# refresh-bio/colord

Hardware: AMD Instinct MI355X
Metric: input Gbases/s + archive size vs ref, ONT 50 Gb at 1/2/4/8 MI355X (higher is better)
Workload: dtype u64

## Files before the change

### colord_amd/csrc/dna.hip

```cpp
#include "common.hpp"
#include <functional>
#include "objects.hpp"
#include "rc_dev.hpp"
#include "rc_check.hpp"
#include "es_format.hpp"
#include <algorithm>
#include <deque>
#include <thread>
#include <chrono>

namespace {
enum { F_READ_TYPE = 0, F_REV_COMP, F_SEEN, F_LEN_BITS, F_LEN_DATA, F_SYMBOLS, F_SYMBOLS_N, F_READ_ID, F_READ_ID_SHORT,
       F_ANCHOR_LEN, F_SKIP_LOCAL, F_SKIP_DISTANT, F_TUPLE_TYPE, N_FAM };
constexpr uint32_t MAX_ALT = 64;

struct FamTab {
	uint32_t n_sym[N_FAM], max_total[N_FAM], adder[N_FAM];
	uint32_t ctx_base[N_FAM + 1];
	uint64_t state_base[N_FAM + 1];
	uint32_t n_ctx[N_FAM];
	int32_t level, T, S;
	uint32_t sym_B;
	uint32_t max_alt;
	uint32_t long_run;
	uint32_t walk_chunk, walk_warm;
};

struct RefStore { const uint64_t* packed; const uint64_t* word_off; const uint32_t* lens; uint32_t n; };
__device__ inline uint32_t ref_at(const RefStore& R, uint32_t id, bool rev, int64_t pos)
{
	if (id >= R.n) return 255;
	const uint32_t len = R.lens[id];
	if (pos < 0 || pos >= (int64_t)len) return 255;
	const uint32_t p = rev ? (len - 1 - (uint32_t)pos) : (uint32_t)pos;
	const uint32_t b = (uint32_t)(R.packed[R.word_off[id] + (p >> 5)] >> (62 - 2 * (p & 31))) & 3u;
	return rev ? 3u - b : b;
}
struct RefCur {
	uint32_t id = 0xffffffffu, len = 0, widx = 0xffffffffu; bool rev = false, ok = false; uint64_t wo = 0, word = 0;
	__device__ inline void set(const RefStore& R, uint32_t nid, bool nrev)
	{
		rev = nrev;
		if (nid == id) return;
		id = nid; widx = 0xffffffffu; ok = nid < R.n;
		if (ok) { len = R.lens[nid]; wo = R.word_off[nid]; }
	}
	__device__ inline uint32_t at(const RefStore& R, int64_t pos)
	{
		if (!ok || pos < 0 || pos >= (int64_t)len) return 255;
		const uint32_t p = rev ? (len - 1 - (uint32_t)pos) : (uint32_t)pos;
		if ((p >> 5) != widx) { widx = p >> 5; word = R.packed[wo + widx]; }
		const uint32_t b = (uint32_t)(word >> (62 - 2 * (p & 31))) & 3u;
		return rev ? 3u - b : b;
	}
};
__device__ inline uint32_t ilog2_(uint64_t x) { return x ? 64u - (uint32_t)__clzll((long long)x) : 0u; }
__device__ inline uint32_t no_bytes_(uint64_t x) { uint32_t r = 1; x >>= 8; for (; x; ++r) x >>= 8; return r; }

template<typename K> struct KeyFmt {
	static __host__ __device__ inline K make(uint32_t gctx, uint32_t payload) { return ((K)gctx << 8) | (K)payload; }
	static __host__ __device__ inline uint32_t ctx(K k) { return (uint32_t)(k >> 8); }
	static __host__ __device__ inline uint32_t payload(K k) { return (uint32_t)k & 0xffu; }
};
__device__ inline uint32_t key_payload(int fam, uint32_t sym, int e1, int e2)
{
	if (fam == F_TUPLE_TYPE)
	{
		const uint32_t x = e1 == 15 ? 0u : e2 == 15 ? (e1 == T_ANCHOR ? 1u : 2u) : e1 == T_ANCHOR ? 3u : e1 == T_DEL ? 4u : 5u;
		return (x << 3) | sym;
	}
	if (fam == F_SYMBOLS) return ((e1 == 15 ? 0u : (uint32_t)e1 + 1u) << 2) | sym;
	return sym;
}
__device__ inline void key_decode(uint32_t fam, uint32_t p, uint32_t& sym, uint32_t& e1, uint32_t& e2)
{
	if (fam == F_TUPLE_TYPE)
	{
		const uint32_t x = p >> 3; sym = p & 7u;
		e1 = x == 0 ? 15u : (x == 1 || x == 3) ? (uint32_t)T_ANCHOR : x == 2 ? (uint32_t)T_SKIP : x == 4 ? (uint32_t)T_DEL : (uint32_t)T_ALT_ID;
		e2 = x == 3 ? (uint32_t)T_MATCH : x == 4 ? (uint32_t)T_SKIP : x == 5 ? (uint32_t)T_MAIN_REF : 15u;
	}
	else if (fam == F_SYMBOLS) { const uint32_t x = p >> 2; sym = p & 3u; e1 = x ? x - 1u : 15u; e2 = 15u; }
	else { sym = p; e1 = e2 = 15u; }
}
__device__ inline uint32_t key_sym_mask(uint32_t fam) { return fam == F_TUPLE_TYPE ? 7u : fam == F_SYMBOLS ? 3u : 0xffu; }

// ... 372 lines not shown
	if (r >= r1) return;
	uint32_t t = es[es_off[r]] >> 4;
	flag[r - r0] = t == T_START_PLAIN ? 0 : t == T_START_PLAIN_N ? 1 : 2;
}

__global__ __launch_bounds__(256) void k_fill_sidx(const uint64_t* __restrict__ sym_off, uint64_t s0, uint32_t r0, uint32_t r1, TripLayoutDev lay, uint32_t* __restrict__ sidx)
{
	const uint32_t r = r0 + blockIdx.x * 4 + (threadIdx.x >> 6);
	if (r >= r1) return;
	const uint32_t lane = threadIdx.x & 63;
	const uint64_t a = sym_off[r] - s0, b = sym_off[r + 1] - s0;
	if (a == b) return;
	const uint32_t part = part_of_read(lay, r), pl = lay.rank ? lay.rank[part] : part;
	const uint64_t gb = lay.group_base[pl >> 6], p0 = lay.part_sym_start[part];
	for (uint64_t i = a + lane; i < b; i += 64) sidx[i] = (uint32_t)trip_slot(gb, pl & 63, i - p0);
}
template<typename K>
__global__ __launch_bounds__(256) void k_dna_plain(const FamTab* __restrict__ ftp, const uint8_t* __restrict__ es, const uint64_t* __restrict__ es_off,
                                                  const uint32_t* __restrict__ es_ntup, const uint8_t* __restrict__ read_flag, const uint32_t* __restrict__ hdr_counts,
                                                  const uint64_t* __restrict__ sym_off, uint32_t r0, uint32_t r1, K* __restrict__ key)
{
	const uint32_t r = r0 + blockIdx.x * 4 + (threadIdx.x >> 6);
	if (r >= r1) return;
	const uint32_t fl = read_flag[r - r0];
	if (fl == 2) return;
	const FamTab& ft = *ftp;
	const uint32_t lane = threadIdx.x & 63;
	const uint8_t* b = es + es_off[r] + 1;
	const uint32_t len = es_ntup[r] - 1;
	const uint64_t off = sym_off[r - r0] + hdr_counts[r - r0];
	const uint32_t S2 = 2 * ft.S; const uint32_t mask = (1u << S2) - 1;
	const uint32_t fam = fl == 0 ? F_SYMBOLS : F_SYMBOLS_N;
	const uint32_t cbase = ft.ctx_base[fam];
	for (uint32_t i = lane; i < len; i += 64)
	{
		uint32_t ctx = mask;
		if (fl == 0)
		{
			const uint32_t n = i < (uint32_t)ft.S ? i : (uint32_t)ft.S;
			for (uint32_t t = n; t >= 1; --t) ctx = ((ctx << 2) + (b[i - t] & 3u)) & mask;
			ctx <<= 2;
		}
		else
		{
			const uint32_t n = i < 4 ? i : 4;
			for (uint32_t t = n; t >= 1; --t) ctx = ((ctx << 4) + (b[i - t] & 0xfu)) & mask;
		}
		key[off + i] = KeyFmt<K>::make(cbase + ctx, b[i] & 0xfu);
	}
}


constexpr uint32_t LONG_RUN = 1u << 19;
struct LongRun { uint32_t s, e, fam, gctx; uint64_t step0, group0, epoch0; uint32_t epoch_cap, pad; };
template<int NS> struct EpochRec { uint32_t start, tot; uint32_t st[NS]; uint32_t cnt0[NS]; };
__device__ inline uint32_t find_run(const LongRun* runs, uint32_t n_runs, uint64_t step)
{
	uint32_t lo = 0, hi = n_runs;
	while (hi - lo > 1) { const uint32_t mid = (lo + hi) >> 1; if (runs[mid].step0 <= step) lo = mid; else hi = mid; }
	return lo;
}
template<typename K>
__global__ void k_long_find(const uint32_t* __restrict__ seg_start, uint32_t n_seg, const K* __restrict__ skey, const FamTab* __restrict__ ftp, LongRun* __restrict__ runs , uint32_t cap, uint32_t* __restrict__ n_runs )
{
	const uint32_t sg = blockIdx.x * blockDim.x + threadIdx.x;
	if (sg >= n_seg) return;
	const uint32_t s = seg_start[sg], e = seg_start[sg + 1];
	const FamTab& ft = *ftp;
	if (e - s < ft.long_run) return;
	const uint32_t gctx = KeyFmt<K>::ctx(skey[s]);
	uint32_t fam = 0;
	for (uint32_t f = 1; f < N_FAM; ++f) if (gctx >= ft.ctx_base[f]) fam = f;
	if (ft.n_sym[fam] > 32) return;
	const uint32_t which = ft.n_sym[fam] > 8 ? 1u : 0u;
	const uint32_t i = atomicAdd(n_runs + which, 1u);
	if (i < cap) { LongRun r; r.s = s; r.e = e; r.fam = fam; r.gctx = gctx; r.step0 = r.group0 = r.epoch0 = 0; r.epoch_cap = 0; r.pad = 0; runs[which * cap + i] = r; }
}
template<int NS, typename K>
__global__ __launch_bounds__(256) void k_long_hist(const LongRun* __restrict__ runs, uint32_t n_runs, uint64_t n_groups, const K* __restrict__ skey,
                                                  uint32_t* __restrict__ step_pfx, uint32_t* __restrict__ group_tot)
{
	const uint64_t g = ((uint64_t)blockIdx.x * blockDim.x + threadIdx.x) >> 6; const uint32_t lane = threadIdx.x & 63;
	if (g >= n_groups) return;
	uint32_t lo = 0, hi = n_runs;
	while (hi - lo > 1) { const uint32_t mid = (lo + hi) >> 1; if (runs[mid].group0 <= g) lo = mid; else hi = mid; }
	const LongRun R = runs[lo];
	const uint64_t gl = g - R.group0;
	const uint32_t smask = key_sym_mask(R.fam);
	uint32_t c[NS];
#pragma unroll
	for (int a = 0; a < NS; ++a) c[a] = 0;
	for (uint32_t k = 0; k < 64; ++k)
	{
		const uint64_t j = (uint64_t)R.s + (gl * 64 + k) * 64 + lane;
		const bool valid = j < R.e;
		const uint32_t sym = valid ? (uint32_t)skey[j] & smask : 0xffu;
#pragma unroll
		for (uint32_t a = 0; a < NS; ++a) { const uint32_t n = (uint32_t)__popcll(__ballot(sym == a)); if (lane == k) c[a] = n; }
	}
	const uint64_t n_steps = ((uint64_t)(R.e - R.s) + 63) / 64;
	const uint64_t step = R.step0 + gl * 64 + lane;
#pragma unroll
	for (uint32_t a = 0; a < NS; ++a)
	{
		const uint32_t incl = wave_incl_scan(c[a]);
		if (gl * 64 + lane < n_steps) step_pfx[step * NS + a] = incl - c[a];
		if (lane == 63) group_tot[g * NS + a] = incl;
	}
}
template<int NS>
__global__ __launch_bounds__(64) void k_long_groups(const LongRun* __restrict__ runs, uint32_t n_runs, uint32_t* __restrict__ group_tot )
{
	const uint32_t r = blockIdx.x, lane = threadIdx.x;
	if (r >= n_runs) return;
	const LongRun R = runs[r];
	const uint64_t n_steps = ((uint64_t)(R.e - R.s) + 63) / 64, n_groups = (n_steps + 63) / 64;
	uint32_t carry[NS];
#pragma unroll
	for (int a = 0; a < NS; ++a) carry[a] = 0;
	for (uint64_t g0 = 0; g0 < n_groups; g0 += 64)
	{
		const uint64_t g = g0 + lane; const bool valid = g < n_groups;
#pragma unroll
		for (uint32_t a = 0; a < NS; ++a)
		{
			const uint32_t v = valid ? group_tot[(R.group0 + g) * NS + a] : 0u;
			const uint32_t incl = wave_incl_scan(v);
			if (valid) group_tot[(R.group0 + g) * NS + a] = carry[a] + incl - v;
			carry[a] += __shfl(incl, 63);
		}
	}
}
template<int NS, typename K>
__device__ inline uint32_t long_prefix(const LongRun& R, const K* skey, const uint32_t* step_pfx, const uint32_t* group_pfx, uint32_t x, uint32_t lane)
{
	const uint32_t smask = key_sym_mask(R.fam);
	const uint64_t step = x >> 6; const uint32_t off = x & 63;
	const uint32_t a = lane & (NS - 1);
	uint32_t v = group_pfx[(R.group0 + (step >> 6)) * NS + a] + (step * 64 < (uint64_t)(R.e - R.s) || off ? step_pfx[(R.step0 + step) * NS + a] : 0u);
	if (x == R.e - R.s && off == 0)
	{
		const uint64_t last = step - 1;
		const uint64_t j = (uint64_t)R.s + last * 64 + lane; const uint32_t sym = j < R.e ? (uint32_t)skey[j] & smask : 0xffu;
		uint32_t mine = 0;
#pragma unroll
		for (uint32_t b = 0; b < NS; ++b) { const uint32_t n = (uint32_t)__popcll(__ballot(sym == b)); if (a == b) mine = n; }
		return group_pfx[(R.group0 + (last >> 6)) * NS + a] + step_pfx[(R.step0 + last) * NS + a] + mine;
	}
	if (off)
	{
		const uint64_t j = (uint64_t)R.s + step * 64 + lane; const uint32_t sym = j < R.e ? (uint32_t)skey[j] & smask : 0xffu;
		const uint64_t below = (1ULL << off) - 1;
		uint32_t mine = 0;
#pragma unroll
		for (uint32_t b = 0; b < NS; ++b) { const uint32_t n = (uint32_t)__popcll(__ballot(sym == b) & below); if (a == b) mine = n; }
		v += mine;
	}
	return v;
}
template<int NS, typename K>
__global__ __launch_bounds__(64) void k_long_epochs(const FamTab* __restrict__ ftp, const LongRun* __restrict__ runs, uint32_t n_runs, const K* __restrict__ skey,
                                                   const uint32_t* __restrict__ step_pfx, const uint32_t* __restrict__ group_pfx, uint32_t* __restrict__ state,
                                                   EpochRec<NS>* __restrict__ epochs, uint32_t* __restrict__ n_epochs, uint32_t* __restrict__ group_epoch, uint32_t* __restrict__ err)
{
	const uint32_t r = blockIdx.x, lane = threadIdx.x;
	if (r >= n_runs) return;
	const LongRun R = runs[r];
	const FamTab& ft = *ftp;
	const uint32_t n_sym = ft.n_sym[R.fam], max_total = ft.max_total[R.fam], adder = ft.adder[R.fam];
	uint32_t* sp = state + ft.state_base[R.fam] + (uint64_t)(R.gctx - ft.ctx_base[R.fam]) * (n_sym + 1);
	const uint32_t L = R.e - R.s;
	uint32_t st = lane < n_sym ? sp[lane] : 0u, tot = sp[n_sym];
	uint32_t cnt0 = 0, p = 0, ne = 0;
	EpochRec<NS>* E = epochs + R.epoch0;
	for (;;)
	{
		if (ne >= R.epoch_cap) { if (lane == 0) atomicOr(err, 8u); break; }
		if (lane < NS) { E[ne].st[lane] = st; E[ne].cnt0[lane] = cnt0; }
		if (lane == 0) { E[ne].start = p; E[ne].tot = tot; }
		++ne;
		const uint32_t rr = (max_total - tot + adder - 1) / adder;
		if ((uint64_t)p + rr > L) break;
		p += rr;
		const uint32_t c1 = long_prefix<NS, K>(R, skey, step_pfx, group_pfx, p, lane);
		st += adder * (c1 - cnt0); cnt0 = c1;
		tot += adder * rr;
		while (tot >= max_total)
		{
			st = (st + 1) / 2;
			uint32_t sm = lane < NS ? st : 0u;
			for (int o = NS / 2; o; o >>= 1) sm += __shfl_xor(sm, o);
			tot = __shfl(sm, 0);
		}
		if (p == L) { if (lane < NS && ne < R.epoch_cap) { E[ne].st[lane] = st; E[ne].cnt0[lane] = cnt0; } if (lane == 0 && ne < R.epoch_cap) { E[ne].start = p; E[ne].tot = tot; } ++ne; break; }
	}
	const uint32_t cl = long_prefix<NS, K>(R, skey, step_pfx, group_pfx, L, lane);
	if (p < L) { st += adder * (cl - cnt0); tot += adder * (L - p); }
	if (lane < n_sym) sp[lane] = st;
	if (lane == 0) { sp[n_sym] = tot; n_epochs[r] = ne; }
	__builtin_amdgcn_s_waitcnt(0);
	__builtin_amdgcn_fence(__ATOMIC_SEQ_CST, "workgroup");
	const uint64_t n_groups = (((uint64_t)L + 63) / 64 + 63) / 64;
	for (uint64_t g0 = 0; g0 < n_groups; g0 += 64)
	{
		const uint64_t g = g0 + lane;
		if (g >= n_groups) continue;
		const uint32_t pos = (uint32_t)(g * 4096);
		uint32_t lo = 0, hi = ne;
		while (hi - lo > 1) { const uint32_t mid = (lo + hi) >> 1; if (E[mid].start <= pos) lo = mid; else hi = mid; }
		group_epoch[R.group0 + g] = lo;
	}
}
template<int NS, typename K>
__global__ __launch_bounds__(256) void k_long_apply(const LongRun* __restrict__ runs, uint32_t n_runs, uint64_t n_steps, const K* __restrict__ skey, const uint32_t* __restrict__ sval,
                                                   const uint32_t* __restrict__ step_pfx, const uint32_t* __restrict__ group_pfx, const EpochRec<NS>* __restrict__ epochs,
                                                   const uint32_t* __restrict__ n_epochs, const uint32_t* __restrict__ group_epoch, const FamTab* __restrict__ ftp, triple_t* __restrict__ trip)
{
	const uint64_t step = ((uint64_t)blockIdx.x * blockDim.x + threadIdx.x) >> 6; const uint32_t lane = threadIdx.x & 63;
	if (step >= n_steps) return;
	const uint32_t ri = find_run(runs, n_runs, step);
	const LongRun R = runs[ri];
	const uint32_t adder = ftp->adder[R.fam];
	const uint64_t sl = step - R.step0;
	const uint32_t x0 = (uint32_t)(sl * 64), x = x0 + lane;
	const uint64_t j = (uint64_t)R.s + x; const bool valid = j < R.e;
	uint32_t sym = 0xffu, e1 = 15u, e2 = 15u;
	if (valid) key_decode(R.fam, KeyFmt<K>::payload(skey[j]), sym, e1, e2);
	uint64_t m[NS];
#pragma unroll
	for (uint32_t a = 0; a < NS; ++a) m[a] = __ballot(sym == a);
	const EpochRec<NS>* E = epochs + R.epoch0; const uint32_t ne = n_epochs[ri];
	uint32_t e = group_epoch[R.group0 + (sl >> 6)];
	while (e + 1 < ne && E[e + 1].start <= x0) ++e;
	uint32_t me = e;
	while (me + 1 < ne && E[me + 1].start <= x) ++me;
	if (!valid) return;
	const EpochRec<NS>& ep = E[me];
	const uint64_t lt = (1ULL << lane) - 1;
	uint32_t cum = 0, freq = 0, excl = 0;
#pragma unroll
	for (uint32_t a = 0; a < NS; ++a)
	{
		const uint32_t pre = group_pfx[(R.group0 + (sl >> 6)) * NS + a] + step_pfx[step * NS + a] + (uint32_t)__popcll(m[a] & lt);
		const uint32_t v = ep.st[a] + adder * (pre - ep.cnt0[a]);
		const bool ex = NS <= 8 && (a == e1 || a == e2);
		if (ex) excl += v;
		if (a < sym && !ex) cum += v;
		if (a == sym) freq = v;
	}
	trip[sval[j]] = pack_triple(cum, freq, ep.tot + adder * (x - ep.start) - excl);
}

template<typename K>
__global__ __launch_bounds__(256) void k_dna_evolve(const FamTab* __restrict__ ftp, const K* __restrict__ skey, const uint32_t* __restrict__ sval,
                                                   const uint32_t* __restrict__ seg_start, uint32_t n_seg, uint32_t* __restrict__ state, triple_t* __restrict__ trip)
{
	__shared__ uint32_t s_cnt[4][256];
	__shared__ uint32_t s_pre[4][256];
	const uint32_t w = threadIdx.x >> 6, lane = threadIdx.x & 63;
	const uint32_t sg = blockIdx.x * 4 + w;
	if (sg >= n_seg) return;
	const uint32_t s = seg_start[sg], e = seg_start[sg + 1];
	const FamTab& ft = *ftp;
	const uint32_t gctx = KeyFmt<K>::ctx(skey[s]);
	uint32_t fam = 0;
	for (uint32_t f = 1; f < N_FAM; ++f) if (gctx >= ft.ctx_base[f]) fam = f;
	const uint32_t n_sym = ft.n_sym[fam], max_total = ft.max_total[fam], adder = ft.adder[fam];
	uint32_t* sp = state + ft.state_base[fam] + (uint64_t)(gctx - ft.ctx_base[fam]) * (n_sym + 1);
	const uint64_t lt = (1ULL << lane) - 1;
	if (n_sym <= 8)
	{
		if (e - s >= ft.long_run) return;
		uint32_t st[8]; uint32_t tot = sp[n_sym];
#pragma unroll
		for (uint32_t a = 0; a < 8; ++a) st[a] = a < n_sym ? sp[a] : 0u;
		for (uint32_t j0 = s; j0 < e; j0 += 64)
		{
			const uint32_t j = j0 + lane; const bool valid = j < e;
			uint32_t sym = 0xffu, e1 = 15u, e2 = 15u;
			if (valid) key_decode(fam, KeyFmt<K>::payload(skey[j]), sym, e1, e2);
			const uint32_t dst = valid ? sval[j] : 0u;
			uint64_t m[8];
#pragma unroll
			for (uint32_t a = 0; a < 8; ++a) m[a] = __ballot(valid && sym == a);
			const uint32_t cnt = (e - j0) < 64 ? (e - j0) : 64;
			uint32_t start = 0;
			while (start < cnt)
			{
				const uint32_t r = (max_total - tot + adder - 1) / adder;
				const uint32_t now = (cnt - start) < r ? (cnt - start) : r;
				const uint64_t win = (now == 64 ? ~0ULL : ((1ULL << now) - 1)) << start;
				if (lane >= start && lane < start + now)
				{
					const uint64_t before = lt & win;
					uint32_t cum = 0, freq = 0, excl = 0;
#pragma unroll
					for (uint32_t a = 0; a < 8; ++a)
					{
						const uint32_t v = st[a] + adder * (uint32_t)__popcll(m[a] & before);
						const bool ex = a == e1 || a == e2;
						if (ex) excl += v;
						if (a < sym && !ex) cum += v;
						if (a == sym) freq = v;
					}
					trip[dst] = pack_triple(cum, freq, tot + adder * (lane - start) - excl);
				}
#pragma unroll
				for (uint32_t a = 0; a < 8; ++a) st[a] += adder * (uint32_t)__popcll(m[a] & win);
				tot += adder * now;
				while (tot >= max_total)
				{
					tot = 0;
#pragma unroll
					for (uint32_t a = 0; a < 8; ++a) { st[a] = (st[a] + 1) / 2; tot += st[a]; }
				}
				start += now;
			}
		}
		if (lane == 0)
		{
			for (uint32_t a = 0; a < n_sym; ++a) sp[a] = st[a];
			sp[n_sym] = tot;
		}
		return;
	}
	if (n_sym <= 32 && e - s >= ft.long_run) return;
	uint32_t* cnt = s_cnt[w]; uint32_t* pre = s_pre[w];
#pragma unroll
	for (uint32_t t = 0; t < 4; ++t) { uint32_t a = lane * 4 + t; cnt[a] = a < n_sym ? sp[a] : 0u; }
	uint32_t tot = sp[n_sym];
	auto rebuild_prefix = [&]() {
		uint32_t v0 = cnt[lane * 4], v1 = cnt[lane * 4 + 1], v2 = cnt[lane * 4 + 2], v3 = cnt[lane * 4 + 3];
		uint32_t sum = v0 + v1 + v2 + v3;
// ... 380 lines not shown
{
	uint32_t v = prev; bool ok = true;
	const uint32_t start = n_reads > 4 ? n_reads - 4 : 0;
	for (uint32_t r = start; r < n_reads; ++r)
	{
		const uint64_t a = es_off[r], b = es_off[r + 1];
		if (a >= b || b > es_bytes) { ok = false; break; }
		const uint32_t t = es[a] >> 4;
		v = ((v << 2) + (t == T_START_PLAIN ? 0u : t == T_START_PLAIN_N ? 1u : 2u)) & 0xff;
	}
	*out = ok ? (unsigned long long)v : ~0ull;
}
}
cl_status cl_dna_batch_types(cl_ctx* ctx, const uint8_t* d_es, const uint64_t* d_es_off, uint32_t n_reads, uint64_t es_bytes, uint32_t prev_types, uint32_t* out)
{
	if (!ctx || !d_es || !d_es_off || !out) return CL_E_INVALID;
	HIP_TRY(ctx, hipSetDevice(ctx->device));
	uint64_t* hs = nullptr; uint64_t* ds = nullptr;
	HIP_TRY(ctx, cl_slot(ctx, 1, &hs, &ds));
	LAUNCH(ctx, k_batch_types, 1, 1, d_es, d_es_off, n_reads, es_bytes, prev_types, (unsigned long long*)ds);
	HIP_TRY(ctx, hipGetLastError());
	HIP_TRY(ctx, hipStreamSynchronize(ctx->stream));
	const uint64_t v = *(volatile uint64_t*)hs;
	if (v == ~0ull) return cl_fail(ctx, CL_E_INVALID, "cl_dna_batch_types: a tuple stream offset of the last reads lies outside the stream");
	*out = (uint32_t)v;
	return CL_OK;
}
void cl_dna_walked_free(DnaWalked* W) { delete W; }
void cl_dna_set_ahead(cl_dna_coder* D, DnaWalked* W) { if (D) D->ahead.reset(W); else delete W; }
cl_status cl_dna_model_read(const cl_dna_coder* D, uint32_t family, uint64_t context, uint32_t* out)
{
	cl_ctx* ctx = D->ctx;
	const FamTab& f = D->ft;
	if (family >= N_FAM || context >= f.n_ctx[family]) return cl_fail(ctx, CL_E_INVALID, "cl_dna_coder_model: no such family or context");
	if (!D->evolved.empty()) return cl_fail(ctx, CL_E_INVALID, "cl_dna_coder_model: a batch evolved ahead has changed the models");
	HIP_TRY(ctx, hipSetDevice(ctx->device));
	HIP_TRY(ctx, hipStreamSynchronize(ctx->stream));
	const uint32_t n = f.n_sym[family] + 1;
	HIP_TRY(ctx, hipMemcpy(out, D->state.p + f.state_base[family] + context * n, (size_t)n * 4, hipMemcpyDeviceToHost));
	return CL_OK;
}
void cl_dna_coder_state(const cl_dna_coder* D, uint32_t* prev_types, uint32_t* read_id) { if (prev_types) *prev_types = D->prev_types; if (read_id) *read_id = D->cur_read_id; }

cl_status cl_dna_walk_ahead(cl_ctx* ctx, cl_dna_coder* D, const cl_reads* refs, const uint8_t* d_es, const uint64_t* d_es_off, const uint32_t* d_es_ntuples, uint32_t n_reads)
{
	if (!ctx || !D || !refs || !d_es || !d_es_off || !d_es_ntuples || !n_reads) return CL_E_INVALID;
	if (!D->next_valid) return cl_fail(ctx, CL_E_INVALID, "cl_dna_walk_ahead: only while a batch is being coded");
	auto W = std::make_unique<DnaWalked>();
	CL_TRY(dna_walk(ctx, D, refs, d_es, d_es_off, d_es_ntuples, n_reads, D->next_prev_types, D->next_read_id, *W));
	D->ahead = std::move(W);
	return CL_OK;
}
void cl_dna_set_before_tail(cl_dna_coder* D, std::function<cl_status()> fn) { if (D) D->before_tail = std::move(fn); }

namespace {
cl_status dna_evolve_batch(cl_ctx* ctx, cl_dna_coder* D, const cl_reads* refs, const uint8_t* d_es, const uint64_t* d_es_off, const uint32_t* d_es_ntuples, uint32_t n_reads,
                           const uint32_t* h_part_bounds, uint32_t n_parts, std::unique_ptr<DnaWalked> Wp, uint32_t prev_types, uint32_t read_id, DnaEvolved& E)
{
	const uint64_t* inv_tab = nullptr;
	CL_TRY(cl_inv_table(ctx, &inv_tab));
	if (Wp && Wp->presorted && (Wp->part_bounds.size() != (size_t)n_parts + 1 || memcmp(Wp->part_bounds.data(), h_part_bounds, ((size_t)n_parts + 1) * 4) != 0)) Wp.reset();
	if (!Wp) { Wp = std::make_unique<DnaWalked>(); CL_TRY(dna_walk(ctx, D, refs, d_es, d_es_off, d_es_ntuples, n_reads, prev_types, read_id, *Wp)); }
	DnaWalked& W = *Wp;
	DevBuf<uint32_t> err; DEV_ALLOC(ctx, err, 1);
	HIP_TRY(ctx, hipMemsetAsync(err.p, 0, 4, ctx->stream));
	E.d_es = d_es; E.n_reads = n_reads; E.prev_types_in = prev_types; E.read_id_in = read_id; E.prev_types_out = W.prev_types_out;
	E.part_bounds.assign(h_part_bounds, h_part_bounds + n_parts + 1);
	uint32_t p0 = 0; size_t gi = 0;
	while (p0 < n_parts)
	{
		std::unique_ptr<DnaGroupPrep> GP;
		if (W.presorted) { if (gi >= W.groups.size() || !W.groups[gi] || W.groups[gi]->p0 != p0) return cl_fail(ctx, CL_E_INVALID, "cl_dna_encode: prepared groups do not match"); GP = std::move(W.groups[gi++]); }
		else { GP = std::make_unique<DnaGroupPrep>(); CL_TRY(dna_group_prepare(ctx, D, W, p0, h_part_bounds, n_parts, *GP)); }
		const uint32_t p1 = GP->p1, np = p1 - p0, ng = (np + 63) / 64;
		const uint64_t s0 = GP->s0, n_syms = GP->n_syms;
		const std::vector<uint32_t>& rank = GP->rank; const std::vector<uint32_t>& plen_r = GP->plen_r;
		auto G = std::make_unique<PendingGroup>(); G->p0 = p0; G->np = np; G->rank = rank; G->n_syms = GP->n_syms;
		G->d_gbase = std::move(GP->d_gbase); G->d_plen = std::move(GP->d_plen);
		DevBuf<uint64_t>& d_gbase = G->d_gbase; DevBuf<uint32_t>& d_plen = G->d_plen; DevBuf<triple_t>& trip = G->trip;
		DEV_ALLOC(ctx, trip, GP->trip_words);
		if (n_syms)
		{
			DevBuf<uint32_t>& sidx = GP->sidx; DevBuf<uint32_t>& seg = GP->seg; const uint64_t n_seg = GP->n_seg;
			auto models = [&](auto* gkey) -> cl_status {
				typedef std::remove_cv_t<std::remove_pointer_t<decltype(gkey)>> K;
				LAUNCHB_NAMED(ctx, "k_dna_evolve", n_syms * (12.0 + sizeof(K)), (k_dna_evolve<K>), grid_for(n_seg, 4), 256, (const FamTab*)D->d_ft.p, (const K*)gkey, (const uint32_t*)sidx.p, (const uint32_t*)seg.p,
					(uint32_t)n_seg, D->state.p, trip.p);
				HIP_TRY(ctx, hipGetLastError());
				for (int which = 0; which < 2; ++which)
				{
					DnaGroupPrep::LongPrep& L = GP->lp[which];
					const uint32_t nlr = L.n_runs, NS = which ? 32 : 8;
					if (!nlr) continue;
					DevBuf<uint32_t> d_ne, group_epoch, epochs;
					DEV_ALLOC(ctx, d_ne, nlr); DEV_ALLOC(ctx, group_epoch, L.groups + 1); DEV_ALLOC(ctx, epochs, (L.eps + 1) * (2 + 2 * NS));
					const LongRun* cr = L.runs.p; const uint64_t steps = L.steps;
					if (which == 0)
					{
						LAUNCH_NAMED(ctx, "k_long_epochs<8>", (k_long_epochs<8, K>), nlr, 64, (const FamTab*)D->d_ft.p, cr, nlr, (const K*)gkey, (const uint32_t*)L.step_pfx.p, (const uint32_t*)L.group_pfx.p,
							D->state.p, (EpochRec<8>*)epochs.p, d_ne.p, group_epoch.p, err.p);
						LAUNCHB_NAMED(ctx, "k_long_apply<8>", steps * 64 * (12.0 + sizeof(K)), (k_long_apply<8, K>), grid_for(steps * 64, 256), 256, cr, nlr, steps, (const K*)gkey, (const uint32_t*)sidx.p,
							(const uint32_t*)L.step_pfx.p, (const uint32_t*)L.group_pfx.p, (const EpochRec<8>*)epochs.p, (const uint32_t*)d_ne.p, (const uint32_t*)group_epoch.p, (const FamTab*)D->d_ft.p, trip.p);
					}
					else
					{
						LAUNCH_NAMED(ctx, "k_long_epochs<32>", (k_long_epochs<32, K>), nlr, 64, (const FamTab*)D->d_ft.p, cr, nlr, (const K*)gkey, (const uint32_t*)L.step_pfx.p, (const uint32_t*)L.group_pfx.p,
							D->state.p, (EpochRec<32>*)epochs.p, d_ne.p, group_epoch.p, err.p);
						LAUNCHB_NAMED(ctx, "k_long_apply<32>", steps * 64 * (12.0 + sizeof(K)), (k_long_apply<32, K>), grid_for(steps * 64, 256), 256, cr, nlr, steps, (const K*)gkey, (const uint32_t*)sidx.p,
							(const uint32_t*)L.step_pfx.p, (const uint32_t*)L.group_pfx.p, (const EpochRec<32>*)epochs.p, (const uint32_t*)d_ne.p, (const uint32_t*)group_epoch.p, (const FamTab*)D->d_ft.p, trip.p);
					}
					HIP_TRY(ctx, hipGetLastError());
					HIP_TRY(ctx, hipStreamSynchronize(ctx->stream));
				}
				return CL_OK;
			};
			if (W.narrow) CL_TRY(models((const uint32_t*)(W.key32.p + s0))); else CL_TRY(models((const uint64_t*)(W.key.p + s0)));
			HIP_TRY(ctx, hipStreamSynchronize(ctx->stream));
		}
		uint32_t herr = 0;
		HIP_TRY(ctx, hipMemcpy(&herr, err.p, 4, hipMemcpyDeviceToHost));
		if (herr & 8) return cl_fail(ctx, CL_E_UNSUPPORTED, "cl_dna_encode: epoch table of a long context run too small");
		if (herr) return cl_fail(ctx, CL_E_UNSUPPORTED, "cl_dna_encode: a read uses more than 64 alternative references");
		if (D->cstreams.size() < 4) { hipStream_t ns = nullptr; HIP_TRY(ctx, cl_stream_create_role(CL_ROLE_CODER, cl_level_to_prio(cl_role_level(CL_ROLE_CODER, 0)), &ns)); D->cstreams.push_back(ns); }
		G->stream = D->cstreams[D->next_cstream++ % D->cstreams.size()];
		G->out_off.resize(np + 1);
		G->out_off[0] = 0;
		for (uint32_t p = 0; p < np; ++p) { uint64_t sy = plen_r[p]; G->out_off[p + 1] = G->out_off[p] + ((sy * 18 + 7) / 8 + sy / 16 + 64 + 7) / 8 * 8; }
		DEV_ALLOC(ctx, G->tmp, G->out_off[np]);
		DEV_ALLOC(ctx, G->d_out_off, np + 1); DEV_ALLOC(ctx, G->d_size, np); DEV_ALLOC(ctx, G->d_dst_off, np);
		HIP_TRY(ctx, hipStreamSynchronize(ctx->stream));
		{
			LaunchOn on(ctx, G->stream);
			G->sync.s = G->stream;
			hipError_t e1 = hipMemcpyAsync(G->d_out_off.p, G->out_off.data(), (np + 1) * 8, hipMemcpyHostToDevice, G->stream);
			LAUNCH_RANGE_CODE(ctx, n_syms * 8.0, ng, (const triple_t*)trip.p, (const uint64_t*)d_gbase.p, (const uint32_t*)d_plen.p, np, G->tmp.p, (const uint64_t*)G->d_out_off.p, G->d_size.p, inv_tab);
			hipError_t e2 = hipGetLastError();
			HIP_TRY(ctx, e1); HIP_TRY(ctx, e2);
		}
		E.groups.push_back(std::move(G));
		p0 = p1;
	}
	return CL_OK;
}
}

cl_status cl_dna_evolve_ahead(cl_ctx* ctx, cl_dna_coder* D, const cl_reads* refs, const uint8_t* d_es, const uint64_t* d_es_off, const uint32_t* d_es_ntuples, uint32_t n_reads,
                              const uint32_t* h_part_bounds, uint32_t n_parts, DnaWalked* W)
{
	std::unique_ptr<DnaWalked> Wp(W);
	if (!ctx || !D || !refs || !d_es || !h_part_bounds || !n_parts || !W) return CL_E_INVALID;
	if (!D->next_valid || D->evolved.size() >= 4) return cl_fail(ctx, CL_E_INVALID, "cl_dna_evolve_ahead: only while a batch is being coded, at most four batches ahead");
	const uint32_t pt = D->evolved.empty() ? D->next_prev_types : D->ahead_prev_types, rid = D->evolved.empty() ? D->next_read_id : D->ahead_read_id;
	if (W->prev_types_in != pt || W->cur_read_id_in != rid || W->d_es != d_es || W->n_reads != n_reads) return cl_fail(ctx, CL_E_INVALID, "cl_dna_evolve_ahead: not the batch that follows");
	auto E = std::make_unique<DnaEvolved>();
	CL_TRY(dna_evolve_batch(ctx, D, refs, d_es, d_es_off, d_es_ntuples, n_reads, h_part_bounds, n_parts, std::move(Wp), pt, rid, *E));
	D->ahead_prev_types = E->prev_types_out; D->ahead_read_id = rid + n_reads;
	D->evolved.push_back(std::move(E));
	return CL_OK;
}

extern "C" cl_status cl_dna_encode(cl_ctx* ctx, cl_dna_coder* D, const cl_reads* refs, const uint8_t* d_es, const uint64_t* d_es_off,
                                   const uint32_t* d_es_ntuples, uint32_t n_reads, const uint32_t* h_part_bounds, uint32_t n_parts,
                                   uint8_t* d_out, uint64_t cap, uint64_t* h_part_sizes, uint64_t* n_out)
{
	if (!ctx || !D || !refs || !d_es || !d_es_off || !d_es_ntuples || !h_part_bounds || !h_part_sizes || !n_out) return cl_fail(ctx, CL_E_INVALID, "cl_dna_encode: null argument");
	HIP_TRY(ctx, hipSetDevice(ctx->device));
	for (uint32_t p = 0; p < n_parts; ++p) if (h_part_bounds[p] > h_part_bounds[p + 1]) return cl_fail(ctx, CL_E_INVALID, "cl_dna_encode: part bounds must ascend");
	if (n_parts && (h_part_bounds[0] != 0 || h_part_bounds[n_parts] != n_reads)) return cl_fail(ctx, CL_E_INVALID, "cl_dna_encode: parts must cover reads [0, n_reads)");
	*n_out = 0;
	if (!n_parts) return CL_OK;
	uint64_t written = 0;
	std::unique_ptr<DnaEvolved> Ep;
	if (!D->evolved.empty()) { Ep = std::move(D->evolved.front()); D->evolved.pop_front(); }
	if (Ep)
	{
		if (Ep->d_es != d_es || Ep->n_reads != n_reads || Ep->prev_types_in != D->prev_types || Ep->read_id_in != D->cur_read_id || Ep->part_bounds.size() != (size_t)n_parts + 1 ||
		    memcmp(Ep->part_bounds.data(), h_part_bounds, ((size_t)n_parts + 1) * 4) != 0)
			return cl_fail(ctx, CL_E_INVALID, "cl_dna_encode: the batch evolved ahead is not the one encoded next");
		D->ahead.reset();
	}
	else
	{
		std::unique_ptr<DnaWalked> Wp;
		if (D->ahead && D->ahead->d_es == d_es && D->ahead->n_reads == n_reads && D->ahead->prev_types_in == D->prev_types && D->ahead->cur_read_id_in == D->cur_read_id) Wp = std::move(D->ahead);
		D->ahead.reset();
		Ep = std::make_unique<DnaEvolved>();
		CL_TRY(dna_evolve_batch(ctx, D, refs, d_es, d_es_off, d_es_ntuples, n_reads, h_part_bounds, n_parts, std::move(Wp), D->prev_types, D->cur_read_id, *Ep));
	}
	DnaEvolved& E = *Ep;
	D->next_prev_types = E.prev_types_out; D->next_read_id = D->cur_read_id + n_reads; D->next_valid = true;
	struct NextOff { cl_dna_coder* D; ~NextOff() { D->next_valid = false; } } next_off{ D };
	auto finish_group = [&](PendingGroup& g) -> cl_status {
		HIP_TRY(ctx, hipStreamSynchronize(g.stream));
		g.sync.s = nullptr;
		std::vector<uint64_t> size_r(g.np);
// ... 36 lines not shown
```

Before: 3.011.

## Restructure long-run apply kernel to process many steps per wave with prefetch

The long-context apply kernel now assigns each wave a block of up to 64 (or 32) consecutive steps within one group instead of one step per wave. It does the run lookup once per wave, preloads the step and group prefix counts into registers with 16-byte loads, and reads them with readlane. Epoch state is advanced incrementally, and key and value loads are software-prefetched in batches of four. Epoch buffer allocation is hoisted ahead of the evolve launch and the per-bucket stream sync is dropped. This cuts redundant binary searches, global prefix reads and host syncs, at the cost of more register pressure and more complex epoch-boundary handling.

```diff
diff --git a/colord_amd/csrc/dna.hip b/colord_amd/csrc/dna.hip
--- a/colord_amd/csrc/dna.hip
+++ b/colord_amd/csrc/dna.hip
@@ -2,6 +2,7 @@
 #include <functional>
 #include "objects.hpp"
 #include "rc_dev.hpp"
+#include "long_idx.hpp"
 #include "rc_check.hpp"
 #include "es_format.hpp"
 #include <algorithm>
@@ -540,9 +541,7 @@
 {
 	const uint64_t g = ((uint64_t)blockIdx.x * blockDim.x + threadIdx.x) >> 6; const uint32_t lane = threadIdx.x & 63;
 	if (g >= n_groups) return;
-	uint32_t lo = 0, hi = n_runs;
-	while (hi - lo > 1) { const uint32_t mid = (lo + hi) >> 1; if (runs[mid].group0 <= g) lo = mid; else hi = mid; }
-	const LongRun R = runs[lo];
+	const LongRun R = runs[long_idx::find_last_le(n_runs, g, [&](uint32_t i) { return runs[i].group0; })];
 	const uint64_t gl = g - R.group0;
 	const uint32_t smask = key_sym_mask(R.fam);
 	uint32_t c[NS];
@@ -669,44 +668,97 @@
 		group_epoch[R.group0 + g] = lo;
 	}
 }
-template<int NS, typename K>
-__global__ __launch_bounds__(256) void k_long_apply(const LongRun* __restrict__ runs, uint32_t n_runs, uint64_t n_steps, const K* __restrict__ skey, const uint32_t* __restrict__ sval,
+constexpr uint32_t LONG_PF = 4;
+constexpr int LONG_SPW_8 = 64, LONG_SPW_32 = 32;
+template<int NS, int SPW, typename K>
+__global__ __launch_bounds__(256) __attribute__((amdgpu_waves_per_eu(NS <= 8 ? 8 : 6))) void k_long_apply(const LongRun* __restrict__ runs, uint32_t n_runs, uint64_t n_groups, const K* __restrict__ skey, const uint32_t* __restrict__ sval,
                                                    const uint32_t* __restrict__ step_pfx, const uint32_t* __restrict__ group_pfx, const EpochRec<NS>* __restrict__ epochs,
                                                    const uint32_t* __restrict__ n_epochs, const uint32_t* __restrict__ group_epoch, const FamTab* __restrict__ ftp, triple_t* __restrict__ trip)
 {
-	const uint64_t step = ((uint64_t)blockIdx.x * blockDim.x + threadIdx.x) >> 6; const uint32_t lane = threadIdx.x & 63;
-	if (step >= n_steps) return;
-	const uint32_t ri = find_run(runs, n_runs, step);
+	static_assert(NS % 4 == 0 && 64 % SPW == 0 && SPW % LONG_PF == 0, "whole 16-byte loads, whole groups, whole batches");
+	constexpr uint32_t WPG = 64 / SPW;
+	const uint64_t w = (uint64_t)blockIdx.x * 4 + (uint32_t)__builtin_amdgcn_readfirstlane((int)(threadIdx.x >> 6)); const uint32_t lane = threadIdx.x & 63;
+	const uint64_t g = w / WPG;
+	if (g >= n_groups) return;
+	const uint32_t ri = (uint32_t)__builtin_amdgcn_readfirstlane((int)long_idx::find_last_le(n_runs, g, [&](uint32_t i) { return runs[i].group0; }));
 	const LongRun R = runs[ri];
-	const uint32_t adder = ftp->adder[R.fam];
-	const uint64_t sl = step - R.step0;
-	const uint32_t x0 = (uint32_t)(sl * 64), x = x0 + lane;
-	const uint64_t j = (uint64_t)R.s + x; const bool valid = j < R.e;
-	uint32_t sym = 0xffu, e1 = 15u, e2 = 15u;
-	if (valid) key_decode(R.fam, KeyFmt<K>::payload(skey[j]), sym, e1, e2);
-	uint64_t m[NS];
-#pragma unroll
-	for (uint32_t a = 0; a < NS; ++a) m[a] = __ballot(sym == a);
-	const EpochRec<NS>* E = epochs + R.epoch0; const uint32_t ne = n_epochs[ri];
-	uint32_t e = group_epoch[R.group0 + (sl >> 6)];
-	while (e + 1 < ne && E[e + 1].start <= x0) ++e;
-	uint32_t me = e;
-	while (me + 1 < ne && E[me + 1].start <= x) ++me;
-	if (!valid) return;
-	const EpochRec<NS>& ep = E[me];
-	const uint64_t lt = (1ULL << lane) - 1;
-	uint32_t cum = 0, freq = 0, excl = 0;
-#pragma unroll
-	for (uint32_t a = 0; a < NS; ++a)
-	{
-		const uint32_t pre = group_pfx[(R.group0 + (sl >> 6)) * NS + a] + step_pfx[step * NS + a] + (uint32_t)__popcll(m[a] & lt);
-		const uint32_t v = ep.st[a] + adder * (pre - ep.cnt0[a]);
-		const bool ex = NS <= 8 && (a == e1 || a == e2);
-		if (ex) excl += v;
-		if (a < sym && !ex) cum += v;
-		if (a == sym) freq = v;
-	}
-	trip[sval[j]] = pack_triple(cum, freq, ep.tot + adder * (x - ep.start) - excl);
+	const uint32_t adder = ftp->adder[R.fam], L = R.e - R.s;
+	uint64_t sl0;
+	const uint32_t nk = long_idx::wave_steps(L, g - R.group0, (uint32_t)(w % WPG), SPW, sl0);
+	if (!nk) return;
+	const uint32_t x0 = (uint32_t)(sl0 * 64);
+	constexpr uint32_t CPL = NS / WPG;
+	static_assert(CPL % 4 == 0, "whole 16-byte loads");
+	uint32_t spv[CPL];
+	{
+		const uint32_t st = lane % SPW, c0 = lane / SPW * CPL;
+		const uint4* sp = (const uint4*)(step_pfx + (R.step0 + sl0 + st) * NS + c0);
+		const uint4* gp = (const uint4*)(group_pfx + g * NS + c0);
+#pragma unroll
+		for (uint32_t q = 0; q < CPL / 4; ++q)
+		{
+			uint4 t = make_uint4(0, 0, 0, 0);
+			if (st < nk) t = sp[q];
+			const uint4 u = gp[q];
+			spv[4 * q] = t.x + u.x; spv[4 * q + 1] = t.y + u.y; spv[4 * q + 2] = t.z + u.z; spv[4 * q + 3] = t.w + u.w;
+		}
+	}
+	const EpochRec<NS>* E = epochs + R.epoch0; const uint32_t ne = (uint32_t)__builtin_amdgcn_readfirstlane((int)n_epochs[ri]);
+	uint32_t e = (uint32_t)__builtin_amdgcn_readfirstlane((int)group_epoch[g]);
+	uint32_t basev = 0, ep_start = 0, ep_tot = 0, nxt = 0;
+	auto load_epoch = [&]() {
+		ep_start = (uint32_t)__builtin_amdgcn_readfirstlane((int)E[e].start); ep_tot = (uint32_t)__builtin_amdgcn_readfirstlane((int)E[e].tot);
+		basev = E[e].st[lane % NS] - adder * E[e].cnt0[lane % NS];
+		nxt = e + 1 < ne ? (uint32_t)__builtin_amdgcn_readfirstlane((int)E[e + 1].start) : 0xffffffffu;
+	};
+	load_epoch();
+	auto fetch = [&](uint32_t k, K& key, uint32_t& dst) {
+		const uint64_t j = (uint64_t)R.s + x0 + (uint64_t)k * 64 + lane;
+		const bool ok = k < nk && lane < long_idx::step_lanes(L, sl0 + k);
+		key = ok ? skey[j] : (K)0; dst = ok ? sval[j] : 0u;
+	};
+	auto step = [&](uint32_t k, K key, uint32_t dst) {
+		const uint32_t xs = x0 + k * 64, x = xs + lane;
+		const bool valid = lane < long_idx::step_lanes(L, sl0 + k);
+		uint32_t sym = 0xffu, e1 = 15u, e2 = 15u;
+		if (valid) key_decode(R.fam, KeyFmt<K>::payload(key), sym, e1, e2);
+		while (nxt <= xs) { ++e; load_epoch(); }
+		uint32_t cum = 0, freq = 0, tot = 0;
+		uint32_t kk = (uint32_t)__builtin_amdgcn_readfirstlane((int)k);
+		for (;;)
+		{
+			asm volatile("" : "+v"(sym), "+s"(kk));
+			uint32_t c = 0, f = 0, excl = 0;
+#pragma unroll
+			for (uint32_t a = 0; a < NS; ++a)
+			{
+				const uint64_t m = __ballot(sym == a);
+				const uint32_t pre = (uint32_t)__builtin_amdgcn_readlane((int)spv[a % CPL], (int)(kk + a / CPL * SPW)) + __builtin_amdgcn_mbcnt_hi((uint32_t)(m >> 32), __builtin_amdgcn_mbcnt_lo((uint32_t)m, 0u));
+				const uint32_t v = (uint32_t)__builtin_amdgcn_readlane((int)basev, (int)a) + adder * pre;
+				const bool ex = NS <= 8 && (a == e1 || a == e2);
+				if (ex) excl += v;
+				if (a < sym && !ex) c += v;
+				if (a == sym) f = v;
+			}
+			if (x >= ep_start) { cum = c; freq = f; tot = ep_tot + adder * (x - ep_start) - excl; }
+			if (nxt - xs > 63) break;
+			++e; load_epoch();
+		}
+		if (valid) trip[dst] = pack_triple(cum, freq, tot);
+	};
+	K kq[LONG_PF]; uint32_t vq[LONG_PF];
+#pragma unroll
+	for (uint32_t u = 0; u < LONG_PF; ++u) fetch(u, kq[u], vq[u]);
+	for (uint32_t kb = 0; kb < nk; kb += LONG_PF)
+	{
+		K kn[LONG_PF]; uint32_t vn[LONG_PF];
+#pragma unroll
+		for (uint32_t u = 0; u < LONG_PF; ++u) fetch(kb + LONG_PF + u, kn[u], vn[u]);
+#pragma unroll
+		for (uint32_t u = 0; u < LONG_PF; ++u) if (kb + u < nk) step(kb + u, kq[u], vq[u]);
+#pragma unroll
+		for (uint32_t u = 0; u < LONG_PF; ++u) { kq[u] = kn[u]; vq[u] = vn[u]; }
+	}
 }
 
 template<typename K>
@@ -1253,35 +1305,39 @@
 		if (n_syms)
 		{
 			DevBuf<uint32_t>& sidx = GP->sidx; DevBuf<uint32_t>& seg = GP->seg; const uint64_t n_seg = GP->n_seg;
+			DevBuf<uint32_t> d_ne[2], group_epoch[2], epochs[2];
 			auto models = [&](auto* gkey) -> cl_status {
 				typedef std::remove_cv_t<std::remove_pointer_t<decltype(gkey)>> K;
+				for (int which = 0; which < 2; ++which)
+				{
+					const DnaGroupPrep::LongPrep& L = GP->lp[which];
+					if (!L.n_runs) continue;
+					DEV_ALLOC(ctx, d_ne[which], L.n_runs); DEV_ALLOC(ctx, group_epoch[which], L.groups + 1); DEV_ALLOC(ctx, epochs[which], (L.eps + 1) * (2 + 2 * (which ? 32 : 8)));
+				}
 				LAUNCHB_NAMED(ctx, "k_dna_evolve", n_syms * (12.0 + sizeof(K)), (k_dna_evolve<K>), grid_for(n_seg, 4), 256, (const FamTab*)D->d_ft.p, (const K*)gkey, (const uint32_t*)sidx.p, (const uint32_t*)seg.p,
 					(uint32_t)n_seg, D->state.p, trip.p);
 				HIP_TRY(ctx, hipGetLastError());
 				for (int which = 0; which < 2; ++which)
 				{
 					DnaGroupPrep::LongPrep& L = GP->lp[which];
-					const uint32_t nlr = L.n_runs, NS = which ? 32 : 8;
+					const uint32_t nlr = L.n_runs;
 					if (!nlr) continue;
-					DevBuf<uint32_t> d_ne, group_epoch, epochs;
-					DEV_ALLOC(ctx, d_ne, nlr); DEV_ALLOC(ctx, group_epoch, L.groups + 1); DEV_ALLOC(ctx, epochs, (L.eps + 1) * (2 + 2 * NS));
-					const LongRun* cr = L.runs.p; const uint64_t steps = L.steps;
+					const LongRun* cr = L.runs.p; const uint64_t steps = L.steps, groups = L.groups;
 					if (which == 0)
 					{
 						LAUNCH_NAMED(ctx, "k_long_epochs<8>", (k_long_epochs<8, K>), nlr, 64, (const FamTab*)D->d_ft.p, cr, nlr, (const K*)gkey, (const uint32_t*)L.step_pfx.p, (const uint32_t*)L.group_pfx.p,
-							D->state.p, (EpochRec<8>*)epochs.p, d_ne.p, group_epoch.p, err.p);
-						LAUNCHB_NAMED(ctx, "k_long_apply<8>", steps * 64 * (12.0 + sizeof(K)), (k_long_apply<8, K>), grid_for(steps * 64, 256), 256, cr, nlr, steps, (const K*)gkey, (const uint32_t*)sidx.p,
-							(const uint32_t*)L.step_pfx.p, (const uint32_t*)L.group_pfx.p, (const EpochRec<8>*)epochs.p, (const uint32_t*)d_ne.p, (const uint32_t*)group_epoch.p, (const FamTab*)D->d_ft.p, trip.p);
+							D->state.p, (EpochRec<8>*)epochs[0].p, d_ne[0].p, group_epoch[0].p, err.p);
+						LAUNCHB_NAMED(ctx, "k_long_apply<8>", steps * 64 * (12.0 + sizeof(K)), (k_long_apply<8, LONG_SPW_8, K>), grid_for(groups * (64 / LONG_SPW_8), 4), 256, cr, nlr, groups, (const K*)gkey, (const uint32_t*)sidx.p,
+							(const uint32_t*)L.step_pfx.p, (const uint32_t*)L.group_pfx.p, (const EpochRec<8>*)epochs[0].p, (const uint32_t*)d_ne[0].p, (const uint32_t*)group_epoch[0].p, (const FamTab*)D->d_ft.p, trip.p);
 					}
 					else
 					{
 						LAUNCH_NAMED(ctx, "k_long_epochs<32>", (k_long_epochs<32, K>), nlr, 64, (const FamTab*)D->d_ft.p, cr, nlr, (const K*)gkey, (const uint32_t*)L.step_pfx.p, (const uint32_t*)L.group_pfx.p,
-							D->state.p, (EpochRec<32>*)epochs.p, d_ne.p, group_epoch.p, err.p);
-						LAUNCHB_NAMED(ctx, "k_long_apply<32>", steps * 64 * (12.0 + sizeof(K)), (k_long_apply<32, K>), grid_for(steps * 64, 256), 256, cr, nlr, steps, (const K*)gkey, (const uint32_t*)sidx.p,
-							(const uint32_t*)L.step_pfx.p, (const uint32_t*)L.group_pfx.p, (const EpochRec<32>*)epochs.p, (const uint32_t*)d_ne.p, (const uint32_t*)group_epoch.p, (const FamTab*)D->d_ft.p, trip.p);
+							D->state.p, (EpochRec<32>*)epochs[1].p, d_ne[1].p, group_epoch[1].p, err.p);
+						LAUNCHB_NAMED(ctx, "k_long_apply<32>", steps * 64 * (12.0 + sizeof(K)), (k_long_apply<32, LONG_SPW_32, K>), grid_for(groups * (64 / LONG_SPW_32), 4), 256, cr, nlr, groups, (const K*)gkey, (const uint32_t*)sidx.p,
+							(const uint32_t*)L.step_pfx.p, (const uint32_t*)L.group_pfx.p, (const EpochRec<32>*)epochs[1].p, (const uint32_t*)d_ne[1].p, (const uint32_t*)group_epoch[1].p, (const FamTab*)D->d_ft.p, trip.p);
 					}
 					HIP_TRY(ctx, hipGetLastError());
-					HIP_TRY(ctx, hipStreamSynchronize(ctx->stream));
 				}
 				return CL_OK;
 			};
diff --git a/colord_amd/csrc/long_idx.hpp b/colord_amd/csrc/long_idx.hpp
--- /dev/null
+++ b/colord_amd/csrc/long_idx.hpp
@@ -0,0 +1,32 @@
+#pragma once
+#include <cstdint>
+#if defined(__HIPCC__)
+#define LONG_IDX_HD __host__ __device__
+#else
+#define LONG_IDX_HD
+#endif
+
+namespace long_idx {
+LONG_IDX_HD inline uint64_t steps_of(uint32_t L) { return ((uint64_t)L + 63) / 64; }
+LONG_IDX_HD inline uint64_t groups_of(uint32_t L) { return (steps_of(L) + 63) / 64; }
+template<typename F>
+LONG_IDX_HD inline uint32_t find_last_le(uint32_t n, uint64_t x, F first)
+{
+	uint32_t lo = 0, hi = n;
+	while (hi - lo > 1) { const uint32_t mid = lo + ((hi - lo) >> 1); if (first(mid) <= x) lo = mid; else hi = mid; }
+	return lo;
+}
+LONG_IDX_HD inline uint32_t wave_steps(uint32_t L, uint64_t gl, uint32_t sub, uint32_t spw, uint64_t& first)
+{
+	const uint64_t n = steps_of(L);
+	first = gl * 64 + (uint64_t)sub * spw;
+	if (first >= n) return 0;
+	return (uint32_t)(n - first < spw ? n - first : spw);
+}
+LONG_IDX_HD inline uint32_t step_lanes(uint32_t L, uint64_t sl)
+{
+	const uint64_t x0 = sl * 64;
+	if (x0 >= L) return 0;
+	return (uint32_t)(L - x0 < 64 ? L - x0 : 64);
+}
+}
```

Result: no change. 3.001 (-0.3%).
